# dcharatan/pixelsplat

Hardware: NVIDIA H100
Metric: rendered views/sec fwd+bwd @256x256, 3 gauss/px (higher is better)
Workload: dtype f32

## Files before the change

pixelsplat_b200/csrc/ps_common.cuh:

```cuda
#pragma once
#include <cuda_runtime.h>
#include <stdint.h>

#include "../../include/pixelsplat_b200.h"

namespace ps {

constexpr int kTile = PS_TILE;
constexpr int kTilePixels = kTile * kTile;

struct Geom {
    float *depth;
    int32_t *radii;
    float2 *xy;
    float4 *conic_opacity;
    float4 *rgb;
    ushort4 *rect;
    uint8_t *clamped;
    uint32_t *tile_count;
    uint32_t *tile_start;
    uint32_t *tile_cursor;
    long long *n_instances;
    uint32_t *vis_pairs;
    uint32_t *vis_any;
    float4 *cull;
};

struct ImageState {
    float *final_T;
    uint32_t *n_contrib;
    float *color;
    float4 *run_state;
    float *depth_image;
    float *run_depth;
};

constexpr int kLossSlots = PS_LOSS_SLOTS;
struct LossEpilogue {
    const float *target;
    float *sums;
    const float *grad_scale;
};

constexpr int kMaxSegments = 4;

struct HitLists {
    uint2 *hits;
    uint32_t *run_hits;
};

struct Dims {
    int S, V, P, M, deg, sh_layout, cov_layout, H, W, gx, gy, tiles, sh_basis, segK, hit_lists;
    int depth_mode;
    long long capacity;
};

struct Inputs {
// ... 69 lines not shown
        if (_e != cudaSuccess) {                                                         \
            ps::set_error("launch of %s failed: %s", name, cudaGetErrorString(_e));      \
            return PS_ERR_CUDA;                                                          \
        }                                                                                \
        ps::count_launch();                                                              \
    } while (0)

int launch_preprocess(const Dims &d, const Inputs &in, const Geom &g, cudaStream_t st);
int launch_sh_color(const Dims &d, const Inputs &in, const Geom &g, cudaStream_t st);
int launch_binning(const Dims &d, const Geom &g, unsigned long long *keys,
                   unsigned long long *keys_alt, int sort_impl, int segment_hint, cudaStream_t st);
int launch_composite_forward(const Dims &d, const Inputs &in, const Geom &g,
                             const unsigned long long *keys, const ImageState &img,
                             float *out_color, const LossEpilogue &loss, const HitLists &hl, float *loss_partials,
                             cudaStream_t st);
int launch_composite_backward(const Dims &d, const Inputs &in, const Geom &g,
                              const unsigned long long *keys, const ImageState &img,
                              const float *d_color, const float *d_depth, const ViewGrads &vg,
                              const ViewGrads *records, const LossEpilogue &loss, const HitLists &hl,
                              cudaStream_t st);
int launch_composite_forward_v1(const Dims &d, const Inputs &in, const Geom &g,
                                const unsigned long long *keys, const ImageState &img,
                                float *out_color, cudaStream_t st);
int launch_composite_backward_v1(const Dims &d, const Inputs &in, const Geom &g,
                                 const unsigned long long *keys, const ImageState &img,
                                 const float *d_color, const ViewGrads &vg, cudaStream_t st);
int composite_impl();
int set_composite_option(int which, int value);
int get_composite_option(int which);
int composite_segments(long long tasks);
bool composite_hit_lists(long long capacity);
int launch_preprocess_backward(const Dims &d, const Inputs &in, const Geom &g, const ViewGrads &vg,
                               const ps_raster_grads &out, cudaStream_t st);
int launch_gradient_fill(const Dims &d, const ps_raster_grads &out, cudaStream_t st);

}
```

pixelsplat_b200/csrc/raster_api.cu:

```cuda
#include <cstdarg>
#include <atomic>
#include <cstdio>
#include <cstring>
#include <mutex>

#include "ps_common.cuh"

namespace ps {

static thread_local char g_error[512] = "";

void set_error(const char *fmt, ...) {
    va_list ap;
    va_start(ap, fmt);
    vsnprintf(g_error, sizeof(g_error), fmt, ap);
    va_end(ap);
}

static bool g_timing = false;
static cudaEvent_t g_events[kNumMarks];
static bool g_events_ready = false;
static std::atomic<unsigned long long> g_launches{0};

void count_launch() { g_launches.fetch_add(1, std::memory_order_relaxed); }
// ... 141 lines not shown
    L.off.run_state = take(px * 16 * (kMaxSegments - 1));
    L.off.depth_image = L.off.run_depth = 0;
    if (m.depth_mode) {
        L.off.depth_image = take(px * 4);
        L.off.run_depth = take(px * 4 * (kMaxSegments - 1));
    }
    L.det = g_deterministic != 0;
    L.loss_partials = L.det ? take(vt * 8 * 8) : 0;
    L.sizes.image_bytes = o;
    L.sizes.backward_bytes = align_up(vp * 8) + align_up(vp * 16) + align_up(vp * 16);
    L.records = L.sizes.backward_bytes;
    if (L.det) {
        const size_t nr = (size_t)m.capacity * 8;
        L.sizes.backward_bytes += align_up(nr * 8) + align_up(nr * 16) + align_up(nr * 16);
    }
    return L;
}

static Geom make_geom(const Layout &L, void *geom) {
    char *b = static_cast<char *>(geom);
    Geom g;
    g.depth = reinterpret_cast<float *>(b + L.off.depth);
    g.radii = reinterpret_cast<int32_t *>(b + L.off.radii);
    g.xy = reinterpret_cast<float2 *>(b + L.off.xy);
    g.conic_opacity = reinterpret_cast<float4 *>(b + L.off.conic_opacity);
    g.rgb = reinterpret_cast<float4 *>(b + L.off.rgb);
    g.rect = reinterpret_cast<ushort4 *>(b + L.off.rect);
    g.clamped = reinterpret_cast<uint8_t *>(b + L.off.clamped);
    g.tile_count = reinterpret_cast<uint32_t *>(b + L.off.tile_count);
    g.tile_start = reinterpret_cast<uint32_t *>(b + L.off.tile_start);
    g.tile_cursor = reinterpret_cast<uint32_t *>(b + L.off.tile_cursor);
    g.n_instances = reinterpret_cast<long long *>(b + L.off.n_instances);
    g.vis_pairs = reinterpret_cast<uint32_t *>(b + L.off.vis_pairs);
    g.vis_any = reinterpret_cast<uint32_t *>(b + L.off.vis_any);
    g.cull = reinterpret_cast<float4 *>(b + L.off.cull);
    return g;
}

static ImageState make_image(const Layout &L, void *image) {
    char *b = static_cast<char *>(image);
    ImageState im;
    im.final_T = reinterpret_cast<float *>(b + L.off.final_T);
    im.n_contrib = reinterpret_cast<uint32_t *>(b + L.off.n_contrib);
    im.color = reinterpret_cast<float *>(b + L.off.color);
    im.run_state = reinterpret_cast<float4 *>(b + L.off.run_state);
    im.depth_image = L.off.depth_image ? reinterpret_cast<float *>(b + L.off.depth_image) : nullptr;
    im.run_depth = L.off.run_depth ? reinterpret_cast<float *>(b + L.off.run_depth) : nullptr;
    return im;
}

static int check_common(const ps_raster_desc *desc, const ps_raster_inputs *in, const ps_raster_state *state,
                        const Layout &L, bool backward) {
    const size_t image_bytes = backward && L.det ? L.loss_partials : L.sizes.image_bytes;
    if (!in || !state) { set_error("inputs/state is NULL"); return PS_ERR_INVALID_ARGUMENT; }
    if (!in->means || !in->cov || !in->opacities || !in->sh || !in->viewmatrix || !in->projmatrix ||
        !in->campos || !in->tanfov || !in->background) {
        set_error("a required input pointer is NULL");
        return PS_ERR_INVALID_ARGUMENT;
    }
    if (!state->geom || !state->binning || !state->image) { set_error("a state buffer is NULL"); return PS_ERR_INVALID_ARGUMENT; }
    if (state->geom_bytes < L.sizes.geom_bytes || state->binning_bytes < L.sizes.binning_bytes ||
        state->image_bytes < image_bytes) {
        set_error("state buffers too small: need geom %zu binning %zu image %zu, got %zu %zu %zu",
                  L.sizes.geom_bytes, L.sizes.binning_bytes, image_bytes, state->geom_bytes,
                  state->binning_bytes, state->image_bytes);
        return PS_ERR_INVALID_ARGUMENT;
    }
// ... 171 lines not shown
    rc = check_common(desc, in, state, L, true);
    if (rc) return rc;
    if ((!d_color && !(target && grad_scale)) || !scratch || !grads) {
        set_error("d_color (or target + grad_scale) / scratch / grads is NULL");
        return PS_ERR_INVALID_ARGUMENT;
    }
    const LossEpilogue le{d_color ? nullptr : target, nullptr, d_color ? nullptr : grad_scale};
    if (!grads->d_means || !grads->d_cov || !grads->d_opacities || !grads->d_sh) {
        set_error("a required gradient pointer is NULL");
        return PS_ERR_INVALID_ARGUMENT;
    }
    if (scratch_bytes < L.sizes.backward_bytes || ((uintptr_t)scratch & 15)) {
        set_error("backward scratch too small or misaligned: need %zu, got %zu", L.sizes.backward_bytes, scratch_bytes);
        return PS_ERR_INVALID_ARGUMENT;
    }
    cudaStream_t st = static_cast<cudaStream_t>(stream);
    Dims d = make_dims(desc);
    if (!d_depth) d.depth_mode = 0;
    const Inputs I = make_inputs(in);
    const Geom g = make_geom(L, state->geom);
    const unsigned long long *keys = reinterpret_cast<const unsigned long long *>(static_cast<char *>(state->binning) + L.off.keys);
    const ImageState img = make_image(L, state->image);
    const size_t vp = (size_t)d.S * d.V * d.P;
    char *sb = static_cast<char *>(scratch);
    ViewGrads vg;
    vg.d_mean2d = reinterpret_cast<float2 *>(sb);
    vg.d_conic = reinterpret_cast<float4 *>(sb + align_up(vp * 8));
    vg.d_color = reinterpret_cast<float4 *>(sb + align_up(vp * 8) + align_up(vp * 16));
    ViewGrads rec;
    const size_t nr = (size_t)d.capacity * 8;
    rec.d_mean2d = reinterpret_cast<float2 *>(sb + L.records);
    rec.d_conic = reinterpret_cast<float4 *>(sb + L.records + align_up(nr * 8));
    rec.d_color = reinterpret_cast<float4 *>(sb + L.records + align_up(nr * 8) + align_up(nr * 16));
    SideCtx *sc = nullptr;
    if ((rc = side_ready(sc))) return rc;
    std::lock_guard<std::mutex> enqueue_lock(sc->enqueue);
    mark(kMarkBwdStart, st);
    PS_CUDA_CHECK(cudaEventRecord(sc->fork, st));
    PS_CUDA_CHECK(cudaStreamWaitEvent(sc->side, sc->fork, 0));
    if ((rc = launch_gradient_fill(d, *grads, sc->side))) return rc;
    PS_CUDA_CHECK(cudaEventRecord(sc->join, sc->side));
    PS_CUDA_CHECK(cudaMemsetAsync(scratch, 0, L.sizes.backward_bytes, st));
    mark(kMarkBwdZero, st);
    HitLists hl{nullptr, nullptr};
    if (d.hit_lists) {
        hl.hits = reinterpret_cast<uint2 *>(static_cast<char *>(state->binning) + L.off.block_hits);
        hl.run_hits = reinterpret_cast<uint32_t *>(static_cast<char *>(state->binning) + L.off.run_hits);
    }
    if ((rc = launch_composite_backward(d, I, g, keys, img, d_color, d_depth, vg, L.det ? &rec : nullptr, le, hl, st)))
        return rc;
    mark(kMarkCompositeBwd, st);
    PS_CUDA_CHECK(cudaStreamWaitEvent(st, sc->join, 0));
    if ((rc = launch_preprocess_backward(d, I, g, vg, *grads, st))) return rc;
    mark(kMarkPreprocessBwd, st);
    return PS_OK;
}

extern "C" {

PS_API int ps_raster_backward(const ps_raster_desc *desc, const ps_raster_inputs *in, const ps_raster_state *state,
                              const float *d_color, void *scratch, size_t scratch_bytes,
                              const ps_raster_grads *grads, void *stream) {
    if (!d_color) { set_error("d_color is NULL"); return PS_ERR_INVALID_ARGUMENT; }
    return raster_backward_impl(desc, in, state, d_color, nullptr, nullptr, nullptr, scratch, scratch_bytes, grads,
                                stream);
}

PS_API int ps_raster_backward_loss(const ps_raster_desc *desc, const ps_raster_inputs *in, const ps_raster_state *state,
                                   const float *target, const float *grad_scale, void *scratch, size_t scratch_bytes,
                                   const ps_raster_grads *grads, void *stream) {
    if (!target || !grad_scale) { set_error("target / grad_scale is NULL"); return PS_ERR_INVALID_ARGUMENT; }
    return raster_backward_impl(desc, in, state, nullptr, target, grad_scale, nullptr, scratch, scratch_bytes, grads,
                                stream);
}

PS_API int ps_raster_backward_depth(const ps_raster_desc *desc, const ps_raster_inputs *in, const ps_raster_state *state,
                                    const float *d_color, const float *loss_target, const float *grad_scale,
                                    const float *d_depth, void *scratch, size_t scratch_bytes,
                                    const ps_raster_grads *grads, void *stream) {
    if (!d_depth) { set_error("d_depth is NULL"); return PS_ERR_INVALID_ARGUMENT; }
    if (desc && desc->depth_mode == PS_DEPTH_NONE) {
        set_error("ps_raster_backward_depth needs the depth_mode of a depth forward (got 0)");
        return PS_ERR_INVALID_ARGUMENT;
    }
    if (!d_color && !(loss_target && grad_scale)) { set_error("d_color, or loss_target + grad_scale, is NULL"); return PS_ERR_INVALID_ARGUMENT; }
// ... 6 lines not shown
```

pixelsplat_b200/csrc/raster_preprocess_bwd.cu:

```cuda
#include "ps_common.cuh"
#include "raster_math.cuh"

namespace ps {

constexpr int kPreBwdThreads = 128;

template <bool DEPTH>
__global__ void __launch_bounds__(kPreBwdThreads, DEPTH ? 4 : 5)
k_preprocess_bwd(Dims d, Inputs in, Geom geo, ViewGrads vgr, ps_raster_grads out, int row_stride) {
    extern __shared__ float s_dsh[];
    if (*geo.n_instances > d.capacity) return;
    const long long n = geo.n_instances[3];
    const int lane = threadIdx.x & 31, warp = threadIdx.x >> 5;
    const long long i0 = ((long long)blockIdx.x * kPreBwdThreads) + warp * 32;
    if (i0 >= n) return;
    const long long li = i0 + lane;
    const bool live = li < n;
    const uint32_t sgi = live ? geo.vis_any[li] : 0u;
    const uint32_t scene = sgi / (uint32_t)d.P, g = sgi - scene * (uint32_t)d.P;
    const size_t sg = sgi;
    const int cov_n = d.cov_layout == PS_COV_TRIU6 ? 6 : 9;
    const int sh_n = d.M > 0 ? 3 * d.M : 3;
    const int M = d.M, layout = d.sh_layout;
    float *wrows = s_dsh + (size_t)warp * 32 * row_stride;
    float *row = wrows + lane * row_stride;
    const bool in_place = M > 0 && d.V == 1;
    float *grow = in_place ? row : row + (size_t)kPreBwdThreads * row_stride;

    const int rows_valid = (int)min((long long)32, n - i0);
    if (M > 0) gather_rows_async(in.sh, (unsigned long long)sg, rows_valid, sh_n, wrows, row_stride, lane);

    float mx0 = 0.0f, my0 = 0.0f, mz0 = 0.0f;
    if (live) { mx0 = in.means[3 * sg + 0]; my0 = in.means[3 * sg + 1]; mz0 = in.means[3 * sg + 2]; }
    const float *covp = in.cov + sg * cov_n;

    float dmx = 0.0f, dmy = 0.0f, dmz = 0.0f, dop = 0.0f;
    float dcov[6] = {0.0f, 0.0f, 0.0f, 0.0f, 0.0f, 0.0f};
    float dcol[3] = {0.0f, 0.0f, 0.0f};
    bool sh_written = false, sh_ready = false;

    for (int v = 0; v < d.V; ++v) {
        const int vid = (int)scene * d.V + v;
        const size_t vg = (size_t)vid * d.P + g;
        const bool vis = live && geo.radii[vg] > 0;
        if (live && out.d_means2d && vis) {
            float *m2 = out.d_means2d + 3 * vg;
            const float2 t = vgr.d_mean2d[vg];
            m2[0] = t.x; m2[1] = t.y;
        }
        float gx = 0.0f, gy = 0.0f, gz = 0.0f;
        float4 gcol = make_float4(0.0f, 0.0f, 0.0f, 0.0f);
        const float sc = in.scale ? in.scale[vid] : 1.0f;
        const float px = mx0 * sc, py = my0 * sc, pz = mz0 * sc;
        if (vis) {
        const float *__restrict__ vm = in.view + 16 * vid;
        const float *__restrict__ pm = in.proj + 16 * vid;
        const float tanfovx = in.tanfov[2 * vid], tanfovy = in.tanfov[2 * vid + 1];
        const float focal_x = (float)d.W / (2.0f * tanfovx), focal_y = (float)d.H / (2.0f * tanfovy);
        float s6[6];
        load_cov6(covp, d.cov_layout, sc * sc, s6);
        Cov2D cv;
        compute_cov2d(px, py, pz, s6, vm, focal_x, focal_y, tanfovx, tanfovy, cv);

        const float2 g2 = vgr.d_mean2d[vg];
        const float4 gc = vgr.d_conic[vg];
        gcol = vgr.d_color[vg];
        dop += gc.w;

        const float a = cv.a, b = cv.b, c = cv.c;
        const float denom = a * c - b * b;
        const float denom2inv = 1.0f / (denom * denom + 0.0000001f);
        float dL_da = 0.0f, dL_db = 0.0f, dL_dc = 0.0f;
        const float *m0 = cv.m0, *m1 = cv.m1;
        if (denom2inv != 0.0f) {
            dL_da = denom2inv * (-c * c * gc.x + 2.0f * b * c * gc.y + (denom - a * c) * gc.z);
            dL_dc = denom2inv * (-a * a * gc.z + 2.0f * a * b * gc.y + (denom - a * c) * gc.x);
            dL_db = denom2inv * 2.0f * (b * c * gc.x - (denom + 2.0f * b * b) * gc.y + a * b * gc.z);
            const float s2 = sc * sc;
            dcov[0] += s2 * (m0[0] * m0[0] * dL_da + m0[0] * m1[0] * dL_db + m1[0] * m1[0] * dL_dc);
            dcov[3] += s2 * (m0[1] * m0[1] * dL_da + m0[1] * m1[1] * dL_db + m1[1] * m1[1] * dL_dc);
            dcov[5] += s2 * (m0[2] * m0[2] * dL_da + m0[2] * m1[2] * dL_db + m1[2] * m1[2] * dL_dc);
            dcov[1] += s2 * (2.0f * m0[0] * m0[1] * dL_da + (m0[0] * m1[1] + m0[1] * m1[0]) * dL_db + 2.0f * m1[0] * m1[1] * dL_dc);
// ... 54 lines not shown
                    const int idx = sh_index(layout, M, k, ch);
                    const float coef = row[idx];
                    const float sdl = sh_sign(flip, k, dl[ch]);
                    const float val = Y * sdl;
                    grow[idx] = first ? val : grow[idx] + val;
                    const float cd = coef * sdl;
                    dLda += Ya * cd; dLdb += Yb * cd; dLdc += Yc * cd;
                }
            });
            const float3 dLd = sh_grad_unpermute(d.sh_basis, dLda, dLdb, dLdc);
            const float dLdx = dLd.x, dLdy = dLd.y, dLdz = dLd.z;
            if (first) {
                const int nb = (d.deg + 1) * (d.deg + 1);
                for (int k = nb; k < M; ++k)
                    for (int ch = 0; ch < 3; ++ch) grow[sh_index(layout, M, k, ch)] = 0.0f;
            }
            sh_written = true;
            const float inv3 = 1.0f / (len2 * len);
            gx += ((len2 - ddx * ddx) * dLdx - ddy * ddx * dLdy - ddz * ddx * dLdz) * inv3;
            gy += (-ddx * ddy * dLdx + (len2 - ddy * ddy) * dLdy - ddz * ddy * dLdz) * inv3;
            gz += (-ddx * ddz * dLdx - ddy * ddz * dLdy + (len2 - ddz * ddz) * dLdz) * inv3;
        } else if (vis) {
            dcol[0] += gcol.x; dcol[1] += gcol.y; dcol[2] += gcol.z;
        }
        dmx += gx * sc; dmy += gy * sc; dmz += gz * sc;
        if (DEPTH && vis) {
            const float *__restrict__ vm = in.view + 16 * vid;
            const float dz = vgr.d_color[vg].w * depth_value_grad(d.depth_mode, geo.depth[vg], in.scale, in.near_far, vid);
            dmx += dz * vm[2]; dmy += dz * vm[6]; dmz += dz * vm[10];
        }
    }

    if (live) {
        out.d_means[3 * sg + 0] = dmx; out.d_means[3 * sg + 1] = dmy; out.d_means[3 * sg + 2] = dmz;
        out.d_opacities[sg] = dop;
        float *dc = out.d_cov + sg * cov_n;
        if (d.cov_layout == PS_COV_TRIU6) {
#pragma unroll
            for (int i = 0; i < 6; ++i) dc[i] = dcov[i];
        } else {
            dc[0] = dcov[0]; dc[1] = dcov[1]; dc[2] = dcov[2];
            dc[4] = dcov[3]; dc[5] = dcov[4]; dc[8] = dcov[5];
        }
        if (M == 0) {
            float *dsh = out.d_sh + sg * 3;
            dsh[0] = dcol[0]; dsh[1] = dcol[1]; dsh[2] = dcol[2];
        }
    }
    if (M > 0) {
        __syncwarp();
        const float *gsrc = in_place ? wrows : wrows + (size_t)kPreBwdThreads * row_stride;
        scatter_rows(out.d_sh, (unsigned long long)sg, rows_valid, sh_n, gsrc, row_stride, lane);
    }
}

int launch_gradient_fill(const Dims &d, const ps_raster_grads &out, cudaStream_t st) {
    const size_t sp = (size_t)d.S * d.P;
    PS_CUDA_CHECK(cudaMemsetAsync(out.d_means, 0, sp * 3 * sizeof(float), st));
    PS_CUDA_CHECK(cudaMemsetAsync(out.d_cov, 0, sp * (d.cov_layout == PS_COV_TRIU6 ? 6 : 9) * sizeof(float), st));
    PS_CUDA_CHECK(cudaMemsetAsync(out.d_opacities, 0, sp * sizeof(float), st));
    PS_CUDA_CHECK(cudaMemsetAsync(out.d_sh, 0, sp * (d.M > 0 ? 3 * d.M : 3) * sizeof(float), st));
    if (out.d_means2d)
        PS_CUDA_CHECK(cudaMemsetAsync(out.d_means2d, 0, (size_t)d.S * d.V * d.P * 3 * sizeof(float), st));
    return PS_OK;
}

int launch_preprocess_backward(const Dims &d, const Inputs &in, const Geom &g, const ViewGrads &vg,
                               const ps_raster_grads &out, cudaStream_t st) {
    const int row_stride = d.M > 0 ? ((3 * d.M) | 1) : 1;
    const size_t smem = d.M > 0 ? sizeof(float) * kPreBwdThreads * row_stride * (d.V == 1 ? 1 : 2) : 0;
    static unsigned long long attr_devices = 0;
    if (first_use_on_device(attr_devices)) {
        PS_CUDA_CHECK(cudaFuncSetAttribute(k_preprocess_bwd<false>, cudaFuncAttributeMaxDynamicSharedMemorySize, 96 * 1024));
        PS_CUDA_CHECK(cudaFuncSetAttribute(k_preprocess_bwd<true>, cudaFuncAttributeMaxDynamicSharedMemorySize, 96 * 1024));
    }
    const long long sp = (long long)d.S * d.P;
    const unsigned blocks = (unsigned)((sp + kPreBwdThreads - 1) / kPreBwdThreads);
    if (d.depth_mode)
        k_preprocess_bwd<true><<<blocks, kPreBwdThreads, smem, st>>>(d, in, g, vg, out, row_stride);
    else
        k_preprocess_bwd<false><<<blocks, kPreBwdThreads, smem, st>>>(d, in, g, vg, out, row_stride);
    PS_LAUNCH_CHECK("k_preprocess_bwd");
    return PS_OK;
}

}
```

pixelsplat_b200/csrc/raster_math.cuh:

```cuda
#pragma once
#include <cuda_runtime.h>
#include <stdint.h>

namespace ps {

constexpr float kShC0 = 0.28209479177387814f;
constexpr float kShC1 = 0.4886025119029199f;

struct Cov2D {
    float tx, ty, tz;
    float ctx, cty;
    bool clamp_x, clamp_y;
    float m0[3], m1[3];
    float a, b, c;
};

__device__ __forceinline__ void load_cov6(const float *cov, int layout, float scale2, float s[6]) {
    if (layout == PS_COV_TRIU6) {
#pragma unroll
        for (int i = 0; i < 6; ++i) s[i] = cov[i];
    } else {
        s[0] = cov[0]; s[1] = cov[1]; s[2] = cov[2]; s[3] = cov[4]; s[4] = cov[5]; s[5] = cov[8];
    }
    if (scale2 != 1.0f) {
// ... 142 lines not shown
    constexpr int kBatch = 4;
    for (int r0 = 0; r0 < rows_valid; r0 += kBatch) {
        if (sh_n <= 96) {
            float v[kBatch][3];
#pragma unroll
            for (int q = 0; q < kBatch; ++q) {
                const unsigned long long rs = __shfl_sync(0xffffffffu, row_of_lane, min(r0 + q, 31));
                const float *src = base + rs * (unsigned long long)sh_n;
#pragma unroll
                for (int t = 0; t < 3; ++t) {
                    const int c = lane + 32 * t;
                    v[q][t] = (r0 + q < rows_valid && c < sh_n) ? __ldg(src + c) : 0.0f;
                }
            }
#pragma unroll
            for (int q = 0; q < kBatch; ++q)
#pragma unroll
                for (int t = 0; t < 3; ++t) {
                    const int c = lane + 32 * t;
                    if (r0 + q < rows_valid && c < sh_n) wrows[(r0 + q) * row_stride + c] = v[q][t];
                }
        } else {
            for (int q = 0; q < kBatch; ++q) {
                const unsigned long long rs = __shfl_sync(0xffffffffu, row_of_lane, min(r0 + q, 31));
                if (r0 + q < rows_valid)
                    for (int c = lane; c < sh_n; c += 32)
                        wrows[(r0 + q) * row_stride + c] = __ldg(base + rs * (unsigned long long)sh_n + c);
            }
        }
    }
}

__device__ __forceinline__ void gather_rows_async(const float *__restrict__ base, unsigned long long row_of_lane,
                                                  int rows_valid, int sh_n, float *wrows, int row_stride, int lane) {
    for (int r = 0; r < rows_valid; ++r) {
        const unsigned long long rs = __shfl_sync(0xffffffffu, row_of_lane, r);
        const float *src = base + rs * (unsigned long long)sh_n;
        float *dst = wrows + r * row_stride;
        for (int c = lane; c < sh_n; c += 32) {
            const uint32_t saddr = (uint32_t)__cvta_generic_to_shared(dst + c);
            asm volatile("cp.async.ca.shared.global [%0], [%1], 4;" ::"r"(saddr), "l"(src + c) : "memory");
        }
    }
    asm volatile("cp.async.commit_group;" ::: "memory");
}

__device__ __forceinline__ void gather_rows_wait() {
    asm volatile("cp.async.wait_all;" ::: "memory");
    __syncwarp();
}

__device__ __forceinline__ void scatter_rows(float *__restrict__ base, unsigned long long row_of_lane,
                                             int rows_valid, int sh_n, const float *wrows, int row_stride, int lane) {
    for (int r = 0; r < rows_valid; ++r) {
        const unsigned long long rs = __shfl_sync(0xffffffffu, row_of_lane, r);
        float *__restrict__ dst = base + rs * (unsigned long long)sh_n;
        for (int c = lane; c < sh_n; c += 32) dst[c] = wrows[r * row_stride + c];
    }
}

__device__ __forceinline__ int sh_index(int layout, int M, int k, int ch) {
    return layout == PS_SH_M3 ? k * 3 + ch : ch * M + k;
}

}
```

pixelsplat_b200/csrc/raster_preprocess.cu:

```cuda
#include "ps_common.cuh"
#include "raster_math.cuh"

namespace ps {

constexpr int kPreThreads = 128;

__device__ __forceinline__ void warp_append(bool flag, uint32_t value, uint32_t *list, long long *counter, int lane) {
    const unsigned m = __ballot_sync(0xffffffffu, flag);
    if (m == 0u) return;
    const int leader = __ffs(m) - 1;
    unsigned long long base = 0;
    if (lane == leader)
        base = atomicAdd(reinterpret_cast<unsigned long long *>(counter), (unsigned long long)__popc(m));
    base = __shfl_sync(0xffffffffu, base, leader);
    if (flag) list[base + __popc(m & ((1u << lane) - 1u))] = value;
}

__global__ void __launch_bounds__(kPreThreads)
k_preprocess(Dims d, Inputs in, Geom geo, int use_smem_hist) {
    extern __shared__ uint32_t s_hist[];
    const int hist_n = d.V * d.tiles;
    const int scene = blockIdx.y;
    const int lane = threadIdx.x & 31;
    const int g = blockIdx.x * kPreThreads + threadIdx.x;
    const bool live = g < d.P;
    if (use_smem_hist) {
        for (int i = threadIdx.x; i < hist_n; i += kPreThreads) s_hist[i] = 0;
        __syncthreads();
    }
    const size_t sg = (size_t)scene * d.P + (live ? g : 0);
    float mx0 = 0.0f, my0 = 0.0f, mz0 = 0.0f, opacity = 0.0f;
    if (live) {
        mx0 = in.means[3 * sg + 0]; my0 = in.means[3 * sg + 1]; mz0 = in.means[3 * sg + 2];
        opacity = in.opac[sg];
    }
    const float *covp = in.cov + sg * (d.cov_layout == PS_COV_TRIU6 ? 6 : 9);
    float cov_raw[6];
    {
        float tmp[6] = {0.0f, 0.0f, 0.0f, 0.0f, 0.0f, 0.0f};
        if (live) load_cov6(covp, d.cov_layout, 1.0f, tmp);
#pragma unroll
        for (int i = 0; i < 6; ++i) cov_raw[i] = tmp[i];
    }
    bool any_vis = false;

    for (int v = 0; v < d.V; ++v) {
        const int vid = scene * d.V + v;
        const size_t vg = (size_t)vid * d.P + (live ? g : 0);
        const float *__restrict__ vm = in.view + 16 * vid;
        const float *__restrict__ pm = in.proj + 16 * vid;
        const float sc = in.scale ? in.scale[vid] : 1.0f;
        const float px = in.scale ? mx0 * sc : mx0;
        const float py = in.scale ? my0 * sc : my0;
        const float pz = in.scale ? mz0 * sc : mz0;
        bool vis = live;
        float vz = 0.0f;
        if (vis) {
            geo.radii[vg] = 0;
            vz = vm[2] * px + vm[6] * py + vm[10] * pz + vm[14];
            vis = !(vz <= 0.2f);
        }
        if (vis) {
            const float hx = pm[0] * px + pm[4] * py + pm[8] * pz + pm[12];
            const float hy = pm[1] * px + pm[5] * py + pm[9] * pz + pm[13];
            const float hw = pm[3] * px + pm[7] * py + pm[11] * pz + pm[15];
            const float p_w = 1.0f / (hw + 0.0000001f);
            const float projx = hx * p_w, projy = hy * p_w;
            const float tanfovx = in.tanfov[2 * vid], tanfovy = in.tanfov[2 * vid + 1];
            const float focal_x = (float)d.W / (2.0f * tanfovx);
            const float focal_y = (float)d.H / (2.0f * tanfovy);
            float s6[6];
            {
                const float sc2 = sc * sc;
#pragma unroll
                for (int i = 0; i < 6; ++i) s6[i] = in.scale ? cov_raw[i] * sc2 : cov_raw[i];
            }
            Cov2D cv;
// ... 11 lines not shown
                const int r = (int)my_radius;
                const float rf = (float)r;
                const int minx = min(d.gx, max(0, (int)((pixx - rf) / (float)kTile)));
                const int miny = min(d.gy, max(0, (int)((pixy - rf) / (float)kTile)));
                const int maxx = min(d.gx, max(0, (int)((pixx + rf + (float)(kTile - 1)) / (float)kTile)));
                const int maxy = min(d.gy, max(0, (int)((pixy + rf + (float)(kTile - 1)) / (float)kTile)));
                vis = (maxx - minx) * (maxy - miny) != 0;
                if (vis) {
                    geo.depth[vg] = vz;
                    geo.radii[vg] = r;
                    geo.xy[vg] = make_float2(pixx, pixy);
                    geo.conic_opacity[vg] = make_float4(cv.c * det_inv, -cv.b * det_inv, cv.a * det_inv, opacity);
                    {
                        const float2 ext = cull_extent(cv.a, cv.c, opacity);
                        geo.cull[vg] = make_float4(pixx, pixy, ext.x, ext.y);
                    }
                    geo.rect[vg] = make_ushort4((unsigned short)minx, (unsigned short)miny,
                                                (unsigned short)maxx, (unsigned short)maxy);
                    if (d.M == 0) {
                        const float *__restrict__ col = in.sh + sg * 3;
                        const float dv = d.depth_mode ? depth_value(d.depth_mode, vz, in.scale, in.near_far, vid) : 0.0f;
                        geo.rgb[vg] = make_float4(col[0], col[1], col[2], dv);
                        geo.clamped[vg] = 0;
                    }
                    for (int ty = miny; ty < maxy; ++ty)
                        for (int tx = minx; tx < maxx; ++tx) {
                            const int t = ty * d.gx + tx;
                            if (use_smem_hist) atomicAdd(&s_hist[v * d.tiles + t], 1u);
                            else atomicAdd(&geo.tile_count[(size_t)vid * d.tiles + t], 1u);
                        }
                }
            }
        }
        any_vis |= vis;
        warp_append(vis, (uint32_t)vg, geo.vis_pairs, geo.n_instances + 2, lane);
    }
    warp_append(any_vis, (uint32_t)sg, geo.vis_any, geo.n_instances + 3, lane);
    if (use_smem_hist) {
        __syncthreads();
        uint32_t *dst = geo.tile_count + (size_t)scene * d.V * d.tiles;
        for (int i = threadIdx.x; i < hist_n; i += kPreThreads) {
            const uint32_t c = s_hist[i];
            if (c) atomicAdd(&dst[i], c);
        }
    }
}

constexpr int kShThreads = 128;

__global__ void __launch_bounds__(kShThreads)
k_sh_color(Dims d, Inputs in, Geom geo, int row_stride) {
    extern __shared__ float s_rows[];
    const long long n = geo.n_instances[2];
    const int lane = threadIdx.x & 31, warp = threadIdx.x >> 5;
    const long long i0 = ((long long)blockIdx.x * kShThreads) + warp * 32;
    if (i0 >= n) return;
    const long long i = i0 + lane;
    const bool live = i < n;
    const uint32_t vg = live ? geo.vis_pairs[i] : 0u;
    const uint32_t vid = vg / (uint32_t)d.P, g = vg - vid * (uint32_t)d.P;
    const uint32_t scene = vid / (uint32_t)d.V;
    const size_t sg = (size_t)scene * d.P + g;
    const int sh_n = 3 * d.M;
    float *wrows = s_rows + (size_t)warp * 32 * row_stride;
    gather_rows_async(in.sh, (unsigned long long)sg, (int)min((long long)32, n - i0), sh_n, wrows, row_stride, lane);
    const float sc = in.scale ? in.scale[vid] : 1.0f;
    const float m0 = in.means[3 * sg + 0], m1 = in.means[3 * sg + 1], m2 = in.means[3 * sg + 2];
    const float px = in.scale ? m0 * sc : m0, py = in.scale ? m1 * sc : m1, pz = in.scale ? m2 * sc : m2;
    const float cx = in.campos[3 * vid], cy = in.campos[3 * vid + 1], cz = in.campos[3 * vid + 2];
    const float ddx = px - cx, ddy = py - cy, ddz = pz - cz;
    const float len = sqrtf(ddx * ddx + ddy * ddy + ddz * ddz);
    const float x = ddx / len, y = ddy / len, z = ddz / len;
    gather_rows_wait();
    if (!live) return;
    const float *row = wrows + lane * row_stride;
    float acc[3] = {0.0f, 0.0f, 0.0f};
    const int M = d.M, layout = d.sh_layout;
    const float3 sa = sh_arg(d.sh_basis, x, y, z);
    const uint32_t flip = sh_flip_mask(d.sh_basis);
    sh_for_each(d.deg, sa.x, sa.y, sa.z, [&](int k, float Yk, float, float, float) {
        const float Y = sh_sign(flip, k, Yk);
#pragma unroll
        for (int ch = 0; ch < 3; ++ch) {
            const float c = row[sh_index(layout, M, k, ch)];
            acc[ch] = k == 0 ? Y * c : acc[ch] + Y * c;
        }
    });
    float rgb[3];
    uint8_t clamp_bits = 0;
#pragma unroll
    for (int ch = 0; ch < 3; ++ch) {
        const float a = acc[ch] + 0.5f;
        if (a < 0.0f) clamp_bits |= (uint8_t)(1u << ch);
        rgb[ch] = fmaxf(a, 0.0f);
    }
    const float dv = d.depth_mode ? depth_value(d.depth_mode, geo.depth[vg], in.scale, in.near_far, (int)vid) : 0.0f;
    geo.rgb[vg] = make_float4(rgb[0], rgb[1], rgb[2], dv);
    geo.clamped[vg] = clamp_bits;
// ... 29 lines not shown
```

Baseline: 2739.

## Fuse gradient zero-fill into preprocess backward with per-range compaction and vector stores

Removes the separate memsets of the parameter-gradient buffers that ran on a side stream, along with the fork/join events. Each preprocess-backward block now owns a contiguous range of 384 gaussians. It compacts the visible ones by checking radii across views, computes their gradients, stages the results in shared memory, and writes the whole range, zeros included, with aligned float4 stores. It also writes d_means2d for every element of its range. This saves a full extra write pass over the gradient buffers and some stream synchronisation. In exchange the kernel visits all S*P gaussians instead of only the visible list, needs more shared memory and block-level syncs, and drops to a fixed occupancy of 4 blocks per SM.

```diff
diff --git a/pixelsplat_b200/csrc/ps_common.cuh b/pixelsplat_b200/csrc/ps_common.cuh
--- a/pixelsplat_b200/csrc/ps_common.cuh
+++ b/pixelsplat_b200/csrc/ps_common.cuh
@@ -158,6 +158,5 @@
 bool composite_hit_lists(long long capacity);
 int launch_preprocess_backward(const Dims &d, const Inputs &in, const Geom &g, const ViewGrads &vg,
                                const ps_raster_grads &out, cudaStream_t st);
-int launch_gradient_fill(const Dims &d, const ps_raster_grads &out, cudaStream_t st);
 
 }
diff --git a/pixelsplat_b200/csrc/raster_api.cu b/pixelsplat_b200/csrc/raster_api.cu
--- a/pixelsplat_b200/csrc/raster_api.cu
+++ b/pixelsplat_b200/csrc/raster_api.cu
@@ -435,14 +435,7 @@
     rec.d_mean2d = reinterpret_cast<float2 *>(sb + L.records);
     rec.d_conic = reinterpret_cast<float4 *>(sb + L.records + align_up(nr * 8));
     rec.d_color = reinterpret_cast<float4 *>(sb + L.records + align_up(nr * 8) + align_up(nr * 16));
-    SideCtx *sc = nullptr;
-    if ((rc = side_ready(sc))) return rc;
-    std::lock_guard<std::mutex> enqueue_lock(sc->enqueue);
     mark(kMarkBwdStart, st);
-    PS_CUDA_CHECK(cudaEventRecord(sc->fork, st));
-    PS_CUDA_CHECK(cudaStreamWaitEvent(sc->side, sc->fork, 0));
-    if ((rc = launch_gradient_fill(d, *grads, sc->side))) return rc;
-    PS_CUDA_CHECK(cudaEventRecord(sc->join, sc->side));
     PS_CUDA_CHECK(cudaMemsetAsync(scratch, 0, L.sizes.backward_bytes, st));
     mark(kMarkBwdZero, st);
     HitLists hl{nullptr, nullptr};
@@ -453,7 +446,6 @@
     if ((rc = launch_composite_backward(d, I, g, keys, img, d_color, d_depth, vg, L.det ? &rec : nullptr, le, hl, st)))
         return rc;
     mark(kMarkCompositeBwd, st);
-    PS_CUDA_CHECK(cudaStreamWaitEvent(st, sc->join, 0));
     if ((rc = launch_preprocess_backward(d, I, g, vg, *grads, st))) return rc;
     mark(kMarkPreprocessBwd, st);
     return PS_OK;
diff --git a/pixelsplat_b200/csrc/raster_preprocess_bwd.cu b/pixelsplat_b200/csrc/raster_preprocess_bwd.cu
--- a/pixelsplat_b200/csrc/raster_preprocess_bwd.cu
+++ b/pixelsplat_b200/csrc/raster_preprocess_bwd.cu
@@ -4,30 +4,87 @@
 namespace ps {
 
 constexpr int kPreBwdThreads = 128;
+constexpr int kPreBwdRange = 384;
+constexpr int kPreBwdScalars = 10;
+
+template <class F>
+__device__ __forceinline__ void store_rows(float *__restrict__ dst, int w, int j_lo, int j_hi, F val) {
+    const int e0 = j_lo * w, e1 = j_hi * w;
+    if (e0 >= e1) return;
+    const int head = min((int)((4 - (((uintptr_t)(dst + e0) >> 2) & 3)) & 3), e1 - e0);
+    const int a0 = e0 + head, n4 = (e1 - a0) >> 2, a1 = a0 + 4 * n4;
+    for (int e = e0 + (int)threadIdx.x; e < a0; e += kPreBwdThreads) dst[e] = val(e / w, e % w);
+    for (int q = threadIdx.x; q < n4; q += kPreBwdThreads) {
+        const int e = a0 + 4 * q;
+        int j = e / w, c = e - j * w;
+        float v[4];
+#pragma unroll
+        for (int k = 0; k < 4; ++k) {
+            v[k] = val(j, c);
+            if (++c == w) { c = 0; ++j; }
+        }
+        *reinterpret_cast<float4 *>(dst + e) = make_float4(v[0], v[1], v[2], v[3]);
+    }
+    for (int e = a1 + (int)threadIdx.x; e < e1; e += kPreBwdThreads) dst[e] = val(e / w, e % w);
+}
 
 template <bool DEPTH>
-__global__ void __launch_bounds__(kPreBwdThreads, DEPTH ? 4 : 5)
+__global__ void __launch_bounds__(kPreBwdThreads, 4)
 k_preprocess_bwd(Dims d, Inputs in, Geom geo, ViewGrads vgr, ps_raster_grads out, int row_stride) {
-    extern __shared__ float s_dsh[];
-    if (*geo.n_instances > d.capacity) return;
-    const long long n = geo.n_instances[3];
-    const int lane = threadIdx.x & 31, warp = threadIdx.x >> 5;
-    const long long i0 = ((long long)blockIdx.x * kPreBwdThreads) + warp * 32;
-    if (i0 >= n) return;
-    const long long li = i0 + lane;
-    const bool live = li < n;
-    const uint32_t sgi = live ? geo.vis_any[li] : 0u;
-    const uint32_t scene = sgi / (uint32_t)d.P, g = sgi - scene * (uint32_t)d.P;
-    const size_t sg = sgi;
+    extern __shared__ float s_rows[];
+    __shared__ short s_list[kPreBwdRange];
+    __shared__ short s_slot[kPreBwdRange];
+    __shared__ int s_warp_n[kPreBwdThreads / 32], s_n_on;
+    __shared__ float s_scal[kPreBwdThreads * kPreBwdScalars];
+
+    const long long r0 = (long long)blockIdx.x * kPreBwdRange;
+    const int rn = (int)min((long long)kPreBwdRange, (long long)d.S * d.P - r0);
+    const int tid = threadIdx.x, lane = tid & 31, warp = tid >> 5;
+    const bool truncated = *geo.n_instances > d.capacity;
+
+    int n_found = 0;
+    for (int base = 0; base < rn; base += kPreBwdThreads) {
+        const int j = base + tid;
+        bool on = false;
+        if (j < rn && !truncated) {
+            const uint32_t sgi = (uint32_t)(r0 + j);
+            const uint32_t scene = sgi / (uint32_t)d.P, g = sgi - scene * (uint32_t)d.P;
+            for (int v = 0; v < d.V; ++v) on |= geo.radii[(size_t)(scene * d.V + v) * d.P + g] > 0;
+        }
+        const unsigned ballot = __ballot_sync(0xffffffffu, on);
+        if (lane == 0) s_warp_n[warp] = __popc(ballot);
+        __syncthreads();
+        int before = n_found, total = n_found;
+#pragma unroll
+        for (int w = 0; w < kPreBwdThreads / 32; ++w) {
+            before += w < warp ? s_warp_n[w] : 0;
+            total += s_warp_n[w];
+        }
+        const int pos = before + __popc(ballot & ((1u << lane) - 1u));
+        if (j < rn) s_slot[j] = on ? (short)pos : (short)-1;
+        if (on) s_list[pos] = (short)j;
+        n_found = total;
+        if (tid == 0) s_n_on = n_found;
+        __syncthreads();
+    }
+
     const int cov_n = d.cov_layout == PS_COV_TRIU6 ? 6 : 9;
     const int sh_n = d.M > 0 ? 3 * d.M : 3;
     const int M = d.M, layout = d.sh_layout;
-    float *wrows = s_dsh + (size_t)warp * 32 * row_stride;
+    float *s_grad = s_rows + (M > 0 && d.V > 1 ? (size_t)kPreBwdThreads * row_stride : 0);
+
+    for (int b0 = 0; b0 == 0 || b0 < s_n_on; b0 += kPreBwdThreads) {
+    const int bn = s_n_on - b0;
+    float *wrows = s_rows + (size_t)warp * 32 * row_stride;
     float *row = wrows + lane * row_stride;
-    const bool in_place = M > 0 && d.V == 1;
-    float *grow = in_place ? row : row + (size_t)kPreBwdThreads * row_stride;
-
-    const int rows_valid = (int)min((long long)32, n - i0);
+    float *grow = s_grad + (size_t)tid * row_stride;
+    if (warp * 32 < bn) {
+    const bool live = tid < bn;
+    const uint32_t sgi = live ? (uint32_t)(r0 + s_list[b0 + tid]) : 0u;
+    const uint32_t scene = sgi / (uint32_t)d.P, g = sgi - scene * (uint32_t)d.P;
+    const size_t sg = sgi;
+
+    const int rows_valid = min(32, bn - warp * 32);
     if (M > 0) gather_rows_async(in.sh, (unsigned long long)sg, rows_valid, sh_n, wrows, row_stride, lane);
 
     float mx0 = 0.0f, my0 = 0.0f, mz0 = 0.0f;
@@ -43,11 +100,6 @@
         const int vid = (int)scene * d.V + v;
         const size_t vg = (size_t)vid * d.P + g;
         const bool vis = live && geo.radii[vg] > 0;
-        if (live && out.d_means2d && vis) {
-            float *m2 = out.d_means2d + 3 * vg;
-            const float2 t = vgr.d_mean2d[vg];
-            m2[0] = t.x; m2[1] = t.y;
-        }
         float gx = 0.0f, gy = 0.0f, gz = 0.0f;
         float4 gcol = make_float4(0.0f, 0.0f, 0.0f, 0.0f);
         const float sc = in.scale ? in.scale[vid] : 1.0f;
@@ -168,50 +220,67 @@
     }
 
     if (live) {
-        out.d_means[3 * sg + 0] = dmx; out.d_means[3 * sg + 1] = dmy; out.d_means[3 * sg + 2] = dmz;
-        out.d_opacities[sg] = dop;
-        float *dc = out.d_cov + sg * cov_n;
-        if (d.cov_layout == PS_COV_TRIU6) {
-#pragma unroll
-            for (int i = 0; i < 6; ++i) dc[i] = dcov[i];
-        } else {
-            dc[0] = dcov[0]; dc[1] = dcov[1]; dc[2] = dcov[2];
-            dc[4] = dcov[3]; dc[5] = dcov[4]; dc[8] = dcov[5];
-        }
-        if (M == 0) {
-            float *dsh = out.d_sh + sg * 3;
-            dsh[0] = dcol[0]; dsh[1] = dcol[1]; dsh[2] = dcol[2];
-        }
-    }
-    if (M > 0) {
-        __syncwarp();
-        const float *gsrc = in_place ? wrows : wrows + (size_t)kPreBwdThreads * row_stride;
-        scatter_rows(out.d_sh, (unsigned long long)sg, rows_valid, sh_n, gsrc, row_stride, lane);
-    }
-}
-
-int launch_gradient_fill(const Dims &d, const ps_raster_grads &out, cudaStream_t st) {
-    const size_t sp = (size_t)d.S * d.P;
-    PS_CUDA_CHECK(cudaMemsetAsync(out.d_means, 0, sp * 3 * sizeof(float), st));
-    PS_CUDA_CHECK(cudaMemsetAsync(out.d_cov, 0, sp * (d.cov_layout == PS_COV_TRIU6 ? 6 : 9) * sizeof(float), st));
-    PS_CUDA_CHECK(cudaMemsetAsync(out.d_opacities, 0, sp * sizeof(float), st));
-    PS_CUDA_CHECK(cudaMemsetAsync(out.d_sh, 0, sp * (d.M > 0 ? 3 * d.M : 3) * sizeof(float), st));
-    if (out.d_means2d)
-        PS_CUDA_CHECK(cudaMemsetAsync(out.d_means2d, 0, (size_t)d.S * d.V * d.P * 3 * sizeof(float), st));
-    return PS_OK;
+        float *sc = s_scal + tid * kPreBwdScalars;
+        sc[0] = dmx; sc[1] = dmy; sc[2] = dmz; sc[3] = dop;
+#pragma unroll
+        for (int i = 0; i < 6; ++i) sc[4 + i] = dcov[i];
+        if (M == 0) { grow[0] = dcol[0]; grow[1] = dcol[1]; grow[2] = dcol[2]; }
+    }
+    }
+    __syncthreads();
+
+    const int n_on = s_n_on, n_lanes = min(n_on - b0, kPreBwdThreads);
+    const int j_lo = b0 == 0 ? 0 : s_list[b0];
+    const int j_hi = b0 + kPreBwdThreads < n_on ? s_list[b0 + kPreBwdThreads] : rn;
+    auto lane_of = [&](int j) { const int s = s_slot[j] - b0; return (unsigned)s < (unsigned)n_lanes ? s : -1; };
+    store_rows(out.d_means + 3 * r0, 3, j_lo, j_hi, [&](int j, int c) {
+        const int l = lane_of(j);
+        return l >= 0 ? s_scal[l * kPreBwdScalars + c] : 0.0f;
+    });
+    store_rows(out.d_opacities + r0, 1, j_lo, j_hi, [&](int j, int) {
+        const int l = lane_of(j);
+        return l >= 0 ? s_scal[l * kPreBwdScalars + 3] : 0.0f;
+    });
+    store_rows(out.d_cov + cov_n * r0, cov_n, j_lo, j_hi, [&](int j, int c) {
+        const int u = cov_n == 6 ? c : (c < 3 ? c : c == 4 ? 3 : c == 5 ? 4 : c == 8 ? 5 : -1);
+        const int l = u >= 0 ? lane_of(j) : -1;
+        return l >= 0 ? s_scal[l * kPreBwdScalars + 4 + u] : 0.0f;
+    });
+    store_rows(out.d_sh + sh_n * r0, sh_n, j_lo, j_hi, [&](int j, int c) {
+        const int l = lane_of(j);
+        return l >= 0 ? s_grad[l * row_stride + c] : 0.0f;
+    });
+    __syncthreads();
+    }
+
+    if (out.d_means2d) {
+        const long long P = d.P;
+        for (long long s = r0 / P; s * P < r0 + rn; ++s) {
+            const long long ga = max(r0, s * P) - s * P, gb = min(r0 + rn, (s + 1) * P) - s * P;
+            for (int v = 0; v < d.V; ++v) {
+                const size_t vg0 = (size_t)(s * d.V + v) * d.P + ga;
+                store_rows(out.d_means2d + 3 * vg0, 3, 0, (int)(gb - ga), [&](int j, int c) {
+                    const size_t vg = vg0 + j;
+                    if (truncated || c == 2 || !(geo.radii[vg] > 0)) return 0.0f;
+                    const float2 t = vgr.d_mean2d[vg];
+                    return c == 0 ? t.x : t.y;
+                });
+            }
+        }
+    }
 }
 
 int launch_preprocess_backward(const Dims &d, const Inputs &in, const Geom &g, const ViewGrads &vg,
                                const ps_raster_grads &out, cudaStream_t st) {
-    const int row_stride = d.M > 0 ? ((3 * d.M) | 1) : 1;
-    const size_t smem = d.M > 0 ? sizeof(float) * kPreBwdThreads * row_stride * (d.V == 1 ? 1 : 2) : 0;
+    const int row_stride = d.M > 0 ? ((3 * d.M) | 1) : 3;
+    const size_t smem = sizeof(float) * kPreBwdThreads * row_stride * (d.M > 0 && d.V > 1 ? 2 : 1);
     static unsigned long long attr_devices = 0;
     if (first_use_on_device(attr_devices)) {
         PS_CUDA_CHECK(cudaFuncSetAttribute(k_preprocess_bwd<false>, cudaFuncAttributeMaxDynamicSharedMemorySize, 96 * 1024));
         PS_CUDA_CHECK(cudaFuncSetAttribute(k_preprocess_bwd<true>, cudaFuncAttributeMaxDynamicSharedMemorySize, 96 * 1024));
     }
     const long long sp = (long long)d.S * d.P;
-    const unsigned blocks = (unsigned)((sp + kPreBwdThreads - 1) / kPreBwdThreads);
+    const unsigned blocks = (unsigned)((sp + kPreBwdRange - 1) / kPreBwdRange);
     if (d.depth_mode)
         k_preprocess_bwd<true><<<blocks, kPreBwdThreads, smem, st>>>(d, in, g, vg, out, row_stride);
     else
```

Result: no change. 2764, median of 6 (+0.9%).

## Write zero gradients in preprocess backward instead of separate memset fills

Applied to the files above, without the earlier changes.

Removes the side-stream memsets of all output gradient buffers and the full scratch memset. The preprocess-backward kernel now covers every Gaussian, computing visibility from radii, and writes zeros directly for invisible warps and unused covariance and mean2d entries. A small kernel clears per-pair view gradients only for visible pairs. The vis_any compaction is dropped. The aim is to cut memset bandwidth, launches and cross-stream synchronisation, at the cost of a denser backward grid and extra radii reads per Gaussian.

```diff
diff --git a/pixelsplat_b200/csrc/ps_common.cuh b/pixelsplat_b200/csrc/ps_common.cuh
--- a/pixelsplat_b200/csrc/ps_common.cuh
+++ b/pixelsplat_b200/csrc/ps_common.cuh
@@ -22,7 +22,6 @@
     uint32_t *tile_cursor;
     long long *n_instances;
     uint32_t *vis_pairs;
-    uint32_t *vis_any;
     float4 *cull;
 };
 
@@ -158,6 +157,6 @@
 bool composite_hit_lists(long long capacity);
 int launch_preprocess_backward(const Dims &d, const Inputs &in, const Geom &g, const ViewGrads &vg,
                                const ps_raster_grads &out, cudaStream_t st);
-int launch_gradient_fill(const Dims &d, const ps_raster_grads &out, cudaStream_t st);
+int launch_clear_pair_grads(const Dims &d, const Geom &g, const ViewGrads &vg, cudaStream_t st);
 
 }
diff --git a/pixelsplat_b200/csrc/raster_api.cu b/pixelsplat_b200/csrc/raster_api.cu
--- a/pixelsplat_b200/csrc/raster_api.cu
+++ b/pixelsplat_b200/csrc/raster_api.cu
@@ -197,7 +197,6 @@
     g.tile_cursor = reinterpret_cast<uint32_t *>(b + L.off.tile_cursor);
     g.n_instances = reinterpret_cast<long long *>(b + L.off.n_instances);
     g.vis_pairs = reinterpret_cast<uint32_t *>(b + L.off.vis_pairs);
-    g.vis_any = reinterpret_cast<uint32_t *>(b + L.off.vis_any);
     g.cull = reinterpret_cast<float4 *>(b + L.off.cull);
     return g;
 }
@@ -435,15 +434,9 @@
     rec.d_mean2d = reinterpret_cast<float2 *>(sb + L.records);
     rec.d_conic = reinterpret_cast<float4 *>(sb + L.records + align_up(nr * 8));
     rec.d_color = reinterpret_cast<float4 *>(sb + L.records + align_up(nr * 8) + align_up(nr * 16));
-    SideCtx *sc = nullptr;
-    if ((rc = side_ready(sc))) return rc;
-    std::lock_guard<std::mutex> enqueue_lock(sc->enqueue);
     mark(kMarkBwdStart, st);
-    PS_CUDA_CHECK(cudaEventRecord(sc->fork, st));
-    PS_CUDA_CHECK(cudaStreamWaitEvent(sc->side, sc->fork, 0));
-    if ((rc = launch_gradient_fill(d, *grads, sc->side))) return rc;
-    PS_CUDA_CHECK(cudaEventRecord(sc->join, sc->side));
-    PS_CUDA_CHECK(cudaMemsetAsync(scratch, 0, L.sizes.backward_bytes, st));
+    if ((rc = launch_clear_pair_grads(d, g, vg, st))) return rc;
+    if (L.det) PS_CUDA_CHECK(cudaMemsetAsync(sb + L.records, 0, L.sizes.backward_bytes - L.records, st));
     mark(kMarkBwdZero, st);
     HitLists hl{nullptr, nullptr};
     if (d.hit_lists) {
@@ -453,7 +446,6 @@
     if ((rc = launch_composite_backward(d, I, g, keys, img, d_color, d_depth, vg, L.det ? &rec : nullptr, le, hl, st)))
         return rc;
     mark(kMarkCompositeBwd, st);
-    PS_CUDA_CHECK(cudaStreamWaitEvent(st, sc->join, 0));
     if ((rc = launch_preprocess_backward(d, I, g, vg, *grads, st))) return rc;
     mark(kMarkPreprocessBwd, st);
     return PS_OK;
diff --git a/pixelsplat_b200/csrc/raster_math.cuh b/pixelsplat_b200/csrc/raster_math.cuh
--- a/pixelsplat_b200/csrc/raster_math.cuh
+++ b/pixelsplat_b200/csrc/raster_math.cuh
@@ -198,8 +198,9 @@
 }
 
 __device__ __forceinline__ void gather_rows_async(const float *__restrict__ base, unsigned long long row_of_lane,
-                                                  int rows_valid, int sh_n, float *wrows, int row_stride, int lane) {
-    for (int r = 0; r < rows_valid; ++r) {
+                                                  unsigned rows, int sh_n, float *wrows, int row_stride, int lane) {
+    for (unsigned m = rows; m != 0u; m &= m - 1u) {
+        const int r = __ffs(m) - 1;
         const unsigned long long rs = __shfl_sync(0xffffffffu, row_of_lane, r);
         const float *src = base + rs * (unsigned long long)sh_n;
         float *dst = wrows + r * row_stride;
@@ -216,12 +217,14 @@
     __syncwarp();
 }
 
-__device__ __forceinline__ void scatter_rows(float *__restrict__ base, unsigned long long row_of_lane,
-                                             int rows_valid, int sh_n, const float *wrows, int row_stride, int lane) {
-    for (int r = 0; r < rows_valid; ++r) {
-        const unsigned long long rs = __shfl_sync(0xffffffffu, row_of_lane, r);
-        float *__restrict__ dst = base + rs * (unsigned long long)sh_n;
-        for (int c = lane; c < sh_n; c += 32) dst[c] = wrows[r * row_stride + c];
+__device__ __forceinline__ void store_rows(float *__restrict__ dst, int rows, int sh_n, const float *wrows,
+                                           int row_stride, int lane) {
+    const int dr = 32 / sh_n, dc = 32 - dr * sh_n;
+    int r = lane / sh_n, c = lane - r * sh_n;
+    for (int e = lane; e < rows * sh_n; e += 32) {
+        dst[e] = wrows[r * row_stride + c];
+        r += dr; c += dc;
+        if (c >= sh_n) { c -= sh_n; ++r; }
     }
 }
 
diff --git a/pixelsplat_b200/csrc/raster_preprocess.cu b/pixelsplat_b200/csrc/raster_preprocess.cu
--- a/pixelsplat_b200/csrc/raster_preprocess.cu
+++ b/pixelsplat_b200/csrc/raster_preprocess.cu
@@ -42,7 +42,6 @@
 #pragma unroll
         for (int i = 0; i < 6; ++i) cov_raw[i] = tmp[i];
     }
-    bool any_vis = false;
 
     for (int v = 0; v < d.V; ++v) {
         const int vid = scene * d.V + v;
@@ -120,10 +119,8 @@
                 }
             }
         }
-        any_vis |= vis;
         warp_append(vis, (uint32_t)vg, geo.vis_pairs, geo.n_instances + 2, lane);
     }
-    warp_append(any_vis, (uint32_t)sg, geo.vis_any, geo.n_instances + 3, lane);
     if (use_smem_hist) {
         __syncthreads();
         uint32_t *dst = geo.tile_count + (size_t)scene * d.V * d.tiles;
@@ -151,7 +148,7 @@
     const size_t sg = (size_t)scene * d.P + g;
     const int sh_n = 3 * d.M;
     float *wrows = s_rows + (size_t)warp * 32 * row_stride;
-    gather_rows_async(in.sh, (unsigned long long)sg, (int)min((long long)32, n - i0), sh_n, wrows, row_stride, lane);
+    gather_rows_async(in.sh, (unsigned long long)sg, __ballot_sync(0xffffffffu, live), sh_n, wrows, row_stride, lane);
     const float sc = in.scale ? in.scale[vid] : 1.0f;
     const float m0 = in.means[3 * sg + 0], m1 = in.means[3 * sg + 1], m2 = in.means[3 * sg + 2];
     const float px = in.scale ? m0 * sc : m0, py = in.scale ? m1 * sc : m1, pz = in.scale ? m2 * sc : m2;
diff --git a/pixelsplat_b200/csrc/raster_preprocess_bwd.cu b/pixelsplat_b200/csrc/raster_preprocess_bwd.cu
--- a/pixelsplat_b200/csrc/raster_preprocess_bwd.cu
+++ b/pixelsplat_b200/csrc/raster_preprocess_bwd.cu
@@ -9,29 +9,45 @@
 __global__ void __launch_bounds__(kPreBwdThreads, DEPTH ? 4 : 5)
 k_preprocess_bwd(Dims d, Inputs in, Geom geo, ViewGrads vgr, ps_raster_grads out, int row_stride) {
     extern __shared__ float s_dsh[];
-    if (*geo.n_instances > d.capacity) return;
-    const long long n = geo.n_instances[3];
     const int lane = threadIdx.x & 31, warp = threadIdx.x >> 5;
-    const long long i0 = ((long long)blockIdx.x * kPreBwdThreads) + warp * 32;
-    if (i0 >= n) return;
-    const long long li = i0 + lane;
-    const bool live = li < n;
-    const uint32_t sgi = live ? geo.vis_any[li] : 0u;
+    const long long sp = (long long)d.S * d.P;
+    const long long sg0 = ((long long)blockIdx.x * kPreBwdThreads) + warp * 32;
+    if (sg0 >= sp) return;
+    const int rows = (int)min((long long)32, sp - sg0);
+    const bool live = lane < rows;
+    const uint32_t sgi = (uint32_t)(live ? sg0 + lane : sg0);
     const uint32_t scene = sgi / (uint32_t)d.P, g = sgi - scene * (uint32_t)d.P;
     const size_t sg = sgi;
     const int cov_n = d.cov_layout == PS_COV_TRIU6 ? 6 : 9;
     const int sh_n = d.M > 0 ? 3 * d.M : 3;
     const int M = d.M, layout = d.sh_layout;
+
+    bool any = false;
+    if (live && *geo.n_instances <= d.capacity)
+        for (int v = 0; v < d.V; ++v) any |= geo.radii[(size_t)((int)scene * d.V + v) * d.P + g] > 0;
+    const unsigned vis_lanes = __ballot_sync(0xffffffffu, any);
+    if (vis_lanes == 0u) {
+        for (int e = lane; e < rows * 3; e += 32) out.d_means[3 * sg0 + e] = 0.0f;
+        for (int e = lane; e < rows * cov_n; e += 32) out.d_cov[cov_n * sg0 + e] = 0.0f;
+        if (lane < rows) out.d_opacities[sg0 + lane] = 0.0f;
+        for (int e = lane; e < rows * sh_n; e += 32) out.d_sh[sh_n * sg0 + e] = 0.0f;
+        if (out.d_means2d && live)
+            for (int v = 0; v < d.V; ++v) {
+                float *m2 = out.d_means2d + 3 * ((size_t)((int)scene * d.V + v) * d.P + g);
+                m2[0] = 0.0f; m2[1] = 0.0f; m2[2] = 0.0f;
+            }
+        return;
+    }
+
     float *wrows = s_dsh + (size_t)warp * 32 * row_stride;
     float *row = wrows + lane * row_stride;
     const bool in_place = M > 0 && d.V == 1;
     float *grow = in_place ? row : row + (size_t)kPreBwdThreads * row_stride;
 
-    const int rows_valid = (int)min((long long)32, n - i0);
-    if (M > 0) gather_rows_async(in.sh, (unsigned long long)sg, rows_valid, sh_n, wrows, row_stride, lane);
+    if (M > 0) gather_rows_async(in.sh, (unsigned long long)sg, vis_lanes, sh_n, wrows, row_stride, lane);
 
     float mx0 = 0.0f, my0 = 0.0f, mz0 = 0.0f;
-    if (live) { mx0 = in.means[3 * sg + 0]; my0 = in.means[3 * sg + 1]; mz0 = in.means[3 * sg + 2]; }
+    if (any) { mx0 = in.means[3 * sg + 0]; my0 = in.means[3 * sg + 1]; mz0 = in.means[3 * sg + 2]; }
     const float *covp = in.cov + sg * cov_n;
 
     float dmx = 0.0f, dmy = 0.0f, dmz = 0.0f, dop = 0.0f;
@@ -42,11 +58,11 @@
     for (int v = 0; v < d.V; ++v) {
         const int vid = (int)scene * d.V + v;
         const size_t vg = (size_t)vid * d.P + g;
-        const bool vis = live && geo.radii[vg] > 0;
-        if (live && out.d_means2d && vis) {
+        const bool vis = any && geo.radii[vg] > 0;
+        if (live && out.d_means2d) {
             float *m2 = out.d_means2d + 3 * vg;
-            const float2 t = vgr.d_mean2d[vg];
-            m2[0] = t.x; m2[1] = t.y;
+            const float2 t = vis ? vgr.d_mean2d[vg] : make_float2(0.0f, 0.0f);
+            m2[0] = t.x; m2[1] = t.y; m2[2] = 0.0f;
         }
         float gx = 0.0f, gy = 0.0f, gz = 0.0f;
         float4 gcol = make_float4(0.0f, 0.0f, 0.0f, 0.0f);
@@ -176,7 +192,8 @@
             for (int i = 0; i < 6; ++i) dc[i] = dcov[i];
         } else {
             dc[0] = dcov[0]; dc[1] = dcov[1]; dc[2] = dcov[2];
-            dc[4] = dcov[3]; dc[5] = dcov[4]; dc[8] = dcov[5];
+            dc[3] = 0.0f; dc[4] = dcov[3]; dc[5] = dcov[4];
+            dc[6] = 0.0f; dc[7] = 0.0f; dc[8] = dcov[5];
         }
         if (M == 0) {
             float *dsh = out.d_sh + sg * 3;
@@ -184,20 +201,29 @@
         }
     }
     if (M > 0) {
+        if (!sh_written)
+            for (int c = 0; c < sh_n; ++c) grow[c] = 0.0f;
         __syncwarp();
         const float *gsrc = in_place ? wrows : wrows + (size_t)kPreBwdThreads * row_stride;
-        scatter_rows(out.d_sh, (unsigned long long)sg, rows_valid, sh_n, gsrc, row_stride, lane);
-    }
-}
-
-int launch_gradient_fill(const Dims &d, const ps_raster_grads &out, cudaStream_t st) {
-    const size_t sp = (size_t)d.S * d.P;
-    PS_CUDA_CHECK(cudaMemsetAsync(out.d_means, 0, sp * 3 * sizeof(float), st));
-    PS_CUDA_CHECK(cudaMemsetAsync(out.d_cov, 0, sp * (d.cov_layout == PS_COV_TRIU6 ? 6 : 9) * sizeof(float), st));
-    PS_CUDA_CHECK(cudaMemsetAsync(out.d_opacities, 0, sp * sizeof(float), st));
-    PS_CUDA_CHECK(cudaMemsetAsync(out.d_sh, 0, sp * (d.M > 0 ? 3 * d.M : 3) * sizeof(float), st));
-    if (out.d_means2d)
-        PS_CUDA_CHECK(cudaMemsetAsync(out.d_means2d, 0, (size_t)d.S * d.V * d.P * 3 * sizeof(float), st));
+        store_rows(out.d_sh + (size_t)sg0 * sh_n, rows, sh_n, gsrc, row_stride, lane);
+    }
+}
+
+constexpr int kClearThreads = 256;
+
+__global__ void __launch_bounds__(kClearThreads) k_clear_pair_grads(Geom geo, ViewGrads vg) {
+    const long long i = (long long)blockIdx.x * kClearThreads + threadIdx.x;
+    if (i >= geo.n_instances[2]) return;
+    const uint32_t p = geo.vis_pairs[i];
+    vg.d_mean2d[p] = make_float2(0.0f, 0.0f);
+    vg.d_conic[p] = make_float4(0.0f, 0.0f, 0.0f, 0.0f);
+    vg.d_color[p] = make_float4(0.0f, 0.0f, 0.0f, 0.0f);
+}
+
+int launch_clear_pair_grads(const Dims &d, const Geom &g, const ViewGrads &vg, cudaStream_t st) {
+    const long long pairs = (long long)d.S * d.V * d.P;
+    k_clear_pair_grads<<<(unsigned)((pairs + kClearThreads - 1) / kClearThreads), kClearThreads, 0, st>>>(g, vg);
+    PS_LAUNCH_CHECK("k_clear_pair_grads");
     return PS_OK;
 }
 
```

Measured after the change: 2752 before, 2978 after (median of 6 runs). 1.08x the previous value.
